# hpcaitech/Open-Sora

Hardware: NVIDIA H100
Metric: denoise-steps/sec STDiT3-XL/2 64x32x32 bf16 (higher is better)
Workload: dtype bf16

## Files before the change

open-sora_b200/csrc/attn_sm90.cu:

```cuda
#include <stdlib.h>

#include "common.cuh"
#include "stage.cuh"
#include "tiles.cuh"
#include "wgmma.cuh"

namespace osb {

constexpr int kAttnThreads = 256;
constexpr int kKeyBlock = 64;

template <int D>
struct FlashState {
  static constexpr int DP = HeadTileCfg<D>::DP;
  uint32_t q[DP / 16][4];
  float o[DP / 8][4];
  float m[2], l[2];
};

template <int D>
__device__ __forceinline__ void flash_load_q(FlashState<D>& f, uint32_t sq, uint32_t chunk_bytes) {
  using Cfg = HeadTileCfg<D>;
  const int lane = threadIdx.x & 31, warp = threadIdx.x >> 5;
  const int row = warp * 16 + (lane & 15);
#pragma unroll
  for (int kk = 0; kk < Cfg::DP / 16; ++kk)
    ldsm_x4(sq + tile_unit_off<Cfg::MAIN>(row, 2 * kk + (lane >> 4), chunk_bytes), f.q[kk][0], f.q[kk][1], f.q[kk][2], f.q[kk][3]);
#pragma unroll
  for (int j = 0; j < Cfg::DP / 8; ++j) f.o[j][0] = f.o[j][1] = f.o[j][2] = f.o[j][3] = 0.f;
  f.m[0] = f.m[1] = -INFINITY;
  f.l[0] = f.l[1] = 0.f;
}

template <int D, bool kBias = false>
__device__ __forceinline__ void flash_block(FlashState<D>& f, uint32_t sk, uint32_t sv, uint32_t chunk_bytes, int krow0,
                                            int n16, int key0, const int (&lo)[2], const int (&hi)[2], float sc,
                                            const float* bias = nullptr, int boff0 = 0, int boff1 = 0, float bscale = 0.f) {
  using Cfg = HeadTileCfg<D>;
  constexpr int NB = kKeyBlock / 8;
  const int lane = threadIdx.x & 31;
  float s[NB][4];
#pragma unroll
  for (int g = 0; g < kKeyBlock / 16; ++g) {
    s[2 * g][0] = s[2 * g][1] = s[2 * g][2] = s[2 * g][3] = 0.f;
    s[2 * g + 1][0] = s[2 * g + 1][1] = s[2 * g + 1][2] = s[2 * g + 1][3] = 0.f;
    if (g >= n16) continue;
    const int krow = krow0 + g * 16 + (lane & 7) + ((lane >> 4) << 3);
#pragma unroll
    for (int kk = 0; kk < Cfg::DP / 16; ++kk) {
      uint32_t b0, b1, b2, b3;
      ldsm_x4(sk + tile_unit_off<Cfg::MAIN>(krow, 2 * kk + ((lane >> 3) & 1), chunk_bytes), b0, b1, b2, b3);
      mma_bf16_16816(s[2 * g], f.q[kk], b0, b1);
      mma_bf16_16816(s[2 * g + 1], f.q[kk], b2, b3);
    }
  }
  float mx[2] = {-INFINITY, -INFINITY};
#pragma unroll
  for (int j = 0; j < NB; ++j) {
#pragma unroll
    for (int e = 0; e < 4; ++e) {
      const int i = e >> 1;
      const int key = key0 + 8 * j + 2 * (lane & 3) + (e & 1);
      if (j >= 2 * n16 || key < lo[i] || key >= hi[i]) s[j][e] = -INFINITY;
      else if constexpr (kBias) s[j][e] = fmaf(s[j][e], bscale, __ldg(bias + key + (i ? boff1 : boff0)));
      mx[i] = fmaxf(mx[i], s[j][e]);
    }
  }
  float alpha[2], ms[2];
#pragma unroll
  for (int i = 0; i < 2; ++i) {
    mx[i] = fmaxf(mx[i], __shfl_xor_sync(0xffffffffu, mx[i], 1));
    mx[i] = fmaxf(mx[i], __shfl_xor_sync(0xffffffffu, mx[i], 2));
    const float mn = fmaxf(f.m[i], mx[i]);
    alpha[i] = (mn == -INFINITY) ? 1.f : fast_exp2((f.m[i] - mn) * sc);
    ms[i] = (mn == -INFINITY) ? 0.f : mn * sc;
    f.m[i] = mn;
    f.l[i] *= alpha[i];
  }
#pragma unroll
  for (int j = 0; j < Cfg::DP / 8; ++j) {
    f.o[j][0] *= alpha[0]; f.o[j][1] *= alpha[0];
    f.o[j][2] *= alpha[1]; f.o[j][3] *= alpha[1];
  }
#pragma unroll
  for (int j = 0; j < NB; ++j) {
#pragma unroll
    for (int e = 0; e < 4; ++e) {
      s[j][e] = fast_exp2(fmaf(s[j][e], sc, -ms[e >> 1]));
      f.l[e >> 1] += s[j][e];
    }
  }
#pragma unroll
  for (int g = 0; g < kKeyBlock / 16; ++g) {
    if (g >= n16) continue;
    const uint32_t a[4] = {pack_bf16x2(s[2 * g][0], s[2 * g][1]), pack_bf16x2(s[2 * g][2], s[2 * g][3]),
                           pack_bf16x2(s[2 * g + 1][0], s[2 * g + 1][1]), pack_bf16x2(s[2 * g + 1][2], s[2 * g + 1][3])};
    const int vrow = krow0 + g * 16 + (lane & 7) + (((lane >> 3) & 1) << 3);
#pragma unroll
    for (int dg = 0; dg < Cfg::DP / 16; ++dg) {
      uint32_t b0, b1, b2, b3;
      ldsm_x4_t(sv + tile_unit_off<Cfg::MAIN>(vrow, 2 * dg + (lane >> 4), chunk_bytes), b0, b1, b2, b3);
      mma_bf16_16816(f.o[2 * dg], a, b0, b1);
      mma_bf16_16816(f.o[2 * dg + 1], a, b2, b3);
    }
  }
}

template <int D>
__device__ __forceinline__ void flash_store(FlashState<D>& f, __nv_bfloat16* dst0, __nv_bfloat16* dst1) {
  const int lane = threadIdx.x & 31;
  float inv[2];
#pragma unroll
  for (int i = 0; i < 2; ++i) {
    float l = f.l[i];
    l += __shfl_xor_sync(0xffffffffu, l, 1);
    l += __shfl_xor_sync(0xffffffffu, l, 2);
    inv[i] = l > 0.f ? 1.0f / l : 0.f;
  }
#pragma unroll
  for (int j = 0; j < D / 8; ++j) {
    const int c = 8 * j + 2 * (lane & 3);
    if (dst0) *reinterpret_cast<uint32_t*>(dst0 + c) = pack_bf16x2(f.o[j][0] * inv[0], f.o[j][1] * inv[0]);
    if (dst1) *reinterpret_cast<uint32_t*>(dst1 + c) = pack_bf16x2(f.o[j][2] * inv[1], f.o[j][3] * inv[1]);
  }
}

struct TileAttnParams {
  const uint8_t* q; const uint8_t* k; const uint8_t* v;
  int64_t q_head_stride, kv_head_stride;
  int32_t q_tile_bytes, kv_tile_bytes;
  int64_t items;
  float scale_log2;
  TileSets ts;
};

template <int D>
struct TileAttnSmem {
  static constexpr int kSlot = 128 * HeadTileCfg<D>::ROW_BYTES;
  static constexpr int kStages = D == 128 ? 2 : (D == 72 ? 4 : 5);
  static constexpr int kData = 2 * kSlot + kStages * 2 * kSlot;
  static constexpr int kBytes = 1024 + kData + 8 * (4 + 2 * kStages);
  static_assert(kBytes <= 227 * 1024 && 2 * kBytes > 228 * 1024, "one resident CTA per SM");
};

constexpr int kTileAttnThreads = 384;

template <int D>
__global__ void __launch_bounds__(kTileAttnThreads, 1) attn_tiles_kernel(const TileAttnParams p) {
  using Cfg = HeadTileCfg<D>;
  using Sm = TileAttnSmem<D>;
  constexpr int MAIN = Cfg::MAIN, TAIL = Cfg::TAIL, STAGES = Sm::kStages;
  extern __shared__ uint8_t smem_raw[];
  const uint32_t base = (smem_u32(smem_raw) + 1023u) & ~1023u;
  auto sQ = [&](int b) { return base + (uint32_t)(b * Sm::kSlot); };
  auto sK = [&](int s) { return base + (uint32_t)((2 + 2 * s) * Sm::kSlot); };
  auto sV = [&](int s) { return sK(s) + (uint32_t)Sm::kSlot; };
  const uint32_t bar = base + (uint32_t)Sm::kData;
  auto q_full = [&](int b) { return bar + 8u * b; };
  auto q_empty = [&](int b) { return bar + 16u + 8u * b; };
  auto full_bar = [&](int s) { return bar + 32u + 8u * s; };
  auto empty_bar = [&](int s) { return bar + 32u + 8u * (STAGES + s); };

  const int wg = threadIdx.x >> 7, tid_wg = threadIdx.x & 127;
  const int64_t begin = (int64_t)blockIdx.x * p.items / gridDim.x, end = (int64_t)(blockIdx.x + 1) * p.items / gridDim.x;
  const TileSets& ts = p.ts;
  const int tps = ts.qmap.tps;

  {
    uint4* z = reinterpret_cast<uint4*>(smem_raw + (base - smem_u32(smem_raw)));
    for (int i = threadIdx.x; i < Sm::kData / 16; i += kTileAttnThreads) z[i] = make_uint4(0, 0, 0, 0);
  }
  fence_proxy_async_smem();
  if (threadIdx.x == 0) {
    for (int b = 0; b < 2; ++b) { mbar_init(q_full(b), 1); mbar_init(q_empty(b), 2); }
    for (int s = 0; s < STAGES; ++s) { mbar_init(full_bar(s), 1); mbar_init(empty_bar(s), 2); }
    fence_barrier_init();
  }
  __syncthreads();
  pdl_wait();

  if (wg == 0) {
    asm volatile("setmaxnreg.dec.sync.aligned.u32 40;\n" ::: "memory");
    if (tid_wg == 0) {
      uint32_t kv_it = 0;
      for (int64_t it = begin; it < end; ++it) {
        const uint32_t n = (uint32_t)(it - begin);
        const int64_t hs = it / tps, head = hs / ts.num_sets, set = hs - head * ts.num_sets;
        const int qs = n & 1;
        mbar_wait_notrace(q_empty(qs), ((n >> 1) & 1u) ^ 1u);
        mbar_expect_tx(q_full(qs), (uint32_t)p.q_tile_bytes);
        bulk_load_1d(sQ(qs), p.q + head * p.q_head_stride + (it - head * ts.num_sets * tps) * p.q_tile_bytes,
                     (uint32_t)p.q_tile_bytes, q_full(qs));
        const int nkt = (tile_set_keys(ts, set) + ts.BK - 1) / ts.BK;
        if (it > begin && (it - 1) / tps == hs && nkt <= STAGES) continue;
        const int64_t off = head * p.kv_head_stride + set * ts.nkb * (int64_t)p.kv_tile_bytes;
        for (int t = 0; t < nkt; ++t, ++kv_it) {
          const int s = (int)(kv_it % STAGES);
          mbar_wait_notrace(empty_bar(s), ((kv_it / STAGES) & 1u) ^ 1u);
          mbar_expect_tx(full_bar(s), 2u * (uint32_t)p.kv_tile_bytes);
          bulk_load_1d(sK(s), p.k + off + (int64_t)t * p.kv_tile_bytes, (uint32_t)p.kv_tile_bytes, full_bar(s));
          bulk_load_1d(sV(s), p.v + off + (int64_t)t * p.kv_tile_bytes, (uint32_t)p.kv_tile_bytes, full_bar(s));
        }
      }
      pdl_launch_dependents();
    }
    return;
  }

  asm volatile("setmaxnreg.inc.sync.aligned.u32 232;\n" ::: "memory");
  const int cw = wg - 1;
  const int lane = tid_wg & 31, quad = lane & 3;
  const int r_loc = cw * 64 + (tid_wg >> 5) * 16 + (lane >> 2);
  const float sc = p.scale_log2;
  float s[64], o[MAIN][32], ot[TAIL ? 8 : 1];
#pragma unroll
  for (int i = 0; i < 64; ++i) s[i] = 0.f;
  uint32_t kv_it = 0, kv0 = 0;
  for (int64_t it = begin; it < end; ++it) {
    const uint32_t n = (uint32_t)(it - begin);
    const int64_t hs = it / tps, head = hs / ts.num_sets, set = hs - head * ts.num_sets;
    const int qt = (int)(it - hs * tps), qs = n & 1;
    const int keys = tile_set_keys(ts, set);
    const int nkt = (keys + ts.BK - 1) / ts.BK;
    if (!(it > begin && (it - 1) / tps == hs && nkt <= STAGES)) { kv0 = kv_it; kv_it += nkt; }
    const bool keep = it + 1 < end && (it + 1) / tps == hs && nkt <= STAGES;

    int64_t seq[2];
    int pos[2], lo[2], hi[2];
    bool valid[2];
#pragma unroll
    for (int hh = 0; hh < 2; ++hh) tile_query_row(ts, set, qt, keys, r_loc + 8 * hh, seq[hh], pos[hh], valid[hh], lo[hh], hi[hh]);
#pragma unroll
    for (int c = 0; c < MAIN; ++c)
#pragma unroll
      for (int i = 0; i < 32; ++i) o[c][i] = 0.f;
#pragma unroll
    for (int i = 0; i < (TAIL ? 8 : 1); ++i) ot[i] = 0.f;
    float m[2] = {-INFINITY, -INFINITY}, l[2] = {0.f, 0.f};

    const uint32_t q_chunk = (uint32_t)ts.qmap.TR * 128u, kv_chunk = (uint32_t)ts.BK * 128u;
    const uint32_t qa = sQ(qs) + (uint32_t)(cw * 64 * 128), qa_tail = sQ(qs) + MAIN * q_chunk + (uint32_t)(cw * 8 * 256);
    mbar_wait_notrace(q_full(qs), (n >> 1) & 1u);
    for (int t = 0; t < nkt; ++t) {
      const uint32_t u = kv0 + (uint32_t)t;
      const int st = (int)(u % STAGES);
      mbar_wait_notrace(full_bar(st), (u / STAGES) & 1u);
      const uint32_t ka = sK(st), va = sV(st);
      wgmma_fence_regs(s);
      wgmma_fence();
#pragma unroll
      for (int c = 0; c < MAIN; ++c)
#pragma unroll
        for (int k = 0; k < 4; ++k)
          Wgmma<128>::mma(s, make_sw128_kmajor_desc(qa + c * q_chunk + 32u * k),
                          make_sw128_kmajor_desc(ka + c * kv_chunk + 32u * k), (c | k) ? 1u : 0u);
      if constexpr (TAIL != 0)
        Wgmma<128>::mma(s, make_noswizzle_desc(qa_tail, 128u, 256u), make_noswizzle_desc(ka + MAIN * kv_chunk, 128u, 256u), 1u);
      wgmma_commit();
      wgmma_wait<0>();
      wgmma_fence_regs(s);
      if (t == nkt - 1 && tid_wg == 0) mbar_arrive(q_empty(qs));
      const int slot0 = t * ts.BK;
      const int n16 = ((keys - slot0 < ts.BK ? keys - slot0 : ts.BK) + 15) >> 4;
      float mx[2] = {-INFINITY, -INFINITY};
#pragma unroll
      for (int i = 0; i < 64; ++i) {
        const int hh = (i >> 1) & 1;
        const int col = 8 * (i >> 2) + 2 * quad + (i & 1), key = slot0 + col;
        if (col >= ts.BK || key < lo[hh] || key >= hi[hh]) s[i] = -INFINITY;
        mx[hh] = fmaxf(mx[hh], s[i]);
      }
      float alpha[2], ms[2];
#pragma unroll
      for (int hh = 0; hh < 2; ++hh) {
        mx[hh] = fmaxf(mx[hh], __shfl_xor_sync(0xffffffffu, mx[hh], 1));
        mx[hh] = fmaxf(mx[hh], __shfl_xor_sync(0xffffffffu, mx[hh], 2));
        const float mn = fmaxf(m[hh], mx[hh]);
        alpha[hh] = (mn == -INFINITY) ? 1.f : fast_exp2((m[hh] - mn) * sc);
        ms[hh] = (mn == -INFINITY) ? 0.f : mn * sc;
        m[hh] = mn;
        l[hh] *= alpha[hh];
      }
#pragma unroll
      for (int c = 0; c < MAIN; ++c)
#pragma unroll
        for (int i = 0; i < 32; ++i) o[c][i] *= alpha[(i >> 1) & 1];
      if constexpr (TAIL != 0) {
#pragma unroll
        for (int i = 0; i < 8; ++i) ot[i] *= alpha[(i >> 1) & 1];
      }
      uint32_t pa[8][4];
#pragma unroll
      for (int i = 0; i < 64; ++i) {
        s[i] = (i >> 3) < n16 ? fast_exp2(fmaf(s[i], sc, -ms[(i >> 1) & 1])) : 0.f;
        l[(i >> 1) & 1] += s[i];
      }
#pragma unroll
      for (int g = 0; g < 8; ++g) {
        pa[g][0] = pack_bf16x2(s[8 * g + 0], s[8 * g + 1]);
        pa[g][1] = pack_bf16x2(s[8 * g + 2], s[8 * g + 3]);
        pa[g][2] = pack_bf16x2(s[8 * g + 4], s[8 * g + 5]);
        pa[g][3] = pack_bf16x2(s[8 * g + 6], s[8 * g + 7]);
      }
#pragma unroll
      for (int c = 0; c < MAIN; ++c) wgmma_fence_regs(o[c]);
      if constexpr (TAIL != 0) wgmma_fence_regs(ot);
      wgmma_fence();
#pragma unroll
      for (int g = 0; g < 8; ++g) {
#pragma unroll
        for (int c = 0; c < MAIN; ++c)
          WgmmaRegAT<64>::mma(o[c], pa[g], make_sw128_kmajor_desc(va + c * kv_chunk + 2048u * g), 1u);
        if constexpr (TAIL != 0)
          WgmmaRegAT<16>::mma(ot, pa[g], make_noswizzle_desc(va + MAIN * kv_chunk + 512u * g, 256u, 128u), 1u);
      }
      wgmma_commit();
      wgmma_wait<0>();
#pragma unroll
      for (int c = 0; c < MAIN; ++c) wgmma_fence_regs(o[c]);
      if constexpr (TAIL != 0) wgmma_fence_regs(ot);
#pragma unroll
      for (int g = 0; g < 8; ++g) fence_regs_u32(pa[g]);
      if (!keep && tid_wg == 0) mbar_arrive(empty_bar(st));
    }
    if (nkt == 0 && tid_wg == 0) mbar_arrive(q_empty(qs));

#pragma unroll
    for (int hh = 0; hh < 2; ++hh) {
      float lt = l[hh];
      lt += __shfl_xor_sync(0xffffffffu, lt, 1);
      lt += __shfl_xor_sync(0xffffffffu, lt, 2);
      const float inv = lt > 0.f ? 1.0f / lt : 0.f;
      if (!valid[hh]) continue;
      __nv_bfloat16* dst = tile_out_row(ts, seq[hh], pos[hh]) + head * D + 2 * quad;
#pragma unroll
      for (int c = 0; c < MAIN; ++c)
#pragma unroll
        for (int j = 0; j < 8; ++j)
          *reinterpret_cast<uint32_t*>(dst + 64 * c + 8 * j) = pack_bf16x2(o[c][4 * j + 2 * hh] * inv, o[c][4 * j + 2 * hh + 1] * inv);
      if constexpr (TAIL != 0)
        *reinterpret_cast<uint32_t*>(dst + 64 * MAIN) = pack_bf16x2(ot[2 * hh] * inv, ot[2 * hh + 1] * inv);
    }
  }
}

template <int D>
static int attn_tiles_launch(TileAttnParams& p, int H, cudaStream_t stream) {
  using Cfg = HeadTileCfg<D>;
  p.q_tile_bytes = p.ts.qmap.TR * Cfg::ROW_BYTES;
  p.kv_tile_bytes = p.ts.BK * Cfg::ROW_BYTES;
  p.items = (int64_t)H * p.ts.num_sets * p.ts.qmap.tps;
  if (p.items >= (1ll << 31)) { set_error("osb_attn_tiles: problem too large (%lld work items)", (long long)p.items); return OSB_ERR_UNSUPPORTED; }
  const int64_t grid = p.items < sm_count() ? p.items : sm_count();
  cudaLaunchAttribute attr[2];
  cudaLaunchConfig_t cfg = launch_config(dim3((unsigned)grid), dim3(kTileAttnThreads), TileAttnSmem<D>::kBytes, stream, attr);
  OSB_CHECK_CUDA(cudaLaunchKernelEx(&cfg, attn_tiles_kernel<D>, p));
  count_launch();
  return OSB_OK;
}

struct AttnParams {
  const __nv_bfloat16* q; const __nv_bfloat16* k; const __nv_bfloat16* v; __nv_bfloat16* out;
  int64_t q_ld, k_ld, v_ld, out_ld;
  int64_t num_seqs, seqs_per_batch;
  int64_t q_bs, q_ss, q_ts, k_bs, k_ss, k_ts;
  int32_t Lq, Lk;
  const int32_t* kv_lens;
  const __nv_bfloat16* qw; const __nv_bfloat16* kw;
  const __nv_bfloat16* qw2; const __nv_bfloat16* kw2;
  int32_t norm_split;
  float eps;
  const float* cos; const float* sin;
  int32_t rope_half;
  float scale_log2;
  int32_t G;
  int32_t tiles_per_seq;
  const float* bias;
  int64_t bias_hs;
  float scale;
};

template <int D>
__device__ __forceinline__ void stage_row(uint4 (&raw)[HeadTileCfg<D>::U], bool norm, float eps, const __nv_bfloat16* w,
                                          const float* cosr, const float* sinr, bool rope_half, uint8_t* tile,
                                          uint32_t chunk_bytes, int row) {
  using Cfg = HeadTileCfg<D>;
  constexpr int U = Cfg::U;
  norm_rope_row<D, U>(raw, norm, eps, w, cosr, sinr, rope_half);
#pragma unroll
  for (int u = 0; u < Cfg::UP; ++u)
    *reinterpret_cast<uint4*>(tile + tile_unit_off<Cfg::MAIN>(row, u, chunk_bytes)) = u < U ? raw[u] : make_uint4(0, 0, 0, 0);
}

template <int D, bool kBias>
__global__ void __launch_bounds__(kAttnThreads, 1) attn_short_kernel(const AttnParams p) {
  using Cfg = HeadTileCfg<D>;
  constexpr int U = Cfg::U;
  extern __shared__ __align__(1024) uint8_t smem[];
  uint8_t* sQ = smem;
  uint8_t* sK = smem + 128 * Cfg::ROW_BYTES;
  uint8_t* sV = sK + kKeyBlock * Cfg::ROW_BYTES;
  const int tid = threadIdx.x, lane = tid & 31, warp = tid >> 5;
  const int64_t unit = blockIdx.x;
  const int h = blockIdx.y;

  int64_t seq0;
  int qt = 0;
  if (p.G > 1) seq0 = unit * p.G;
  else { seq0 = unit / p.tiles_per_seq; qt = (int)(unit - seq0 * p.tiles_per_seq); }
  auto row_of = [&](int64_t seq, int tok, int64_t bs, int64_t ss, int64_t ts) {
    const int64_t b = seq / p.seqs_per_batch, j = seq - b * p.seqs_per_batch;
    return b * bs + j * ss + (int64_t)tok * ts;
  };

  __shared__ int s_nkeys;
  if (tid == 0) s_nkeys = 0;
  __syncthreads();
  pdl_wait();
  for (int r = tid; r < 128; r += kAttnThreads) {
    const int g = p.G > 1 ? r / p.Lq : 0;
    const int tok = p.G > 1 ? r - g * p.Lq : qt * 128 + r;
    const int64_t seq = seq0 + g;
    uint4 raw[U];
    const bool ok = g < p.G && seq < p.num_seqs && tok < p.Lq;
    if (ok) {
      const uint4* src = reinterpret_cast<const uint4*>(p.q + row_of(seq, tok, p.q_bs, p.q_ss, p.q_ts) * p.q_ld + (int64_t)h * D);
#pragma unroll
      for (int u = 0; u < U; ++u) raw[u] = __ldg(src + u);
    } else {
#pragma unroll
      for (int u = 0; u < U; ++u) raw[u] = make_uint4(0, 0, 0, 0);
    }
    const __nv_bfloat16* w = (p.qw2 != nullptr && tok >= p.norm_split) ? p.qw2 : p.qw;
    const bool rope = ok && p.cos != nullptr;
    stage_row<D>(raw, ok && p.qw != nullptr, p.eps, w, rope ? p.cos + (int64_t)tok * (D / 2) : nullptr,
                 rope ? p.sin + (int64_t)tok * (D / 2) : nullptr, p.rope_half, sQ, 128u * 128u, r);
  }

  int lo[2], hi[2];
  int boff[2] = {0, 0};
  __nv_bfloat16* dst[2] = {nullptr, nullptr};
  int nkeys = 0;
#pragma unroll
  for (int i = 0; i < 2; ++i) {
    const int r = warp * 16 + (lane >> 2) + 8 * i;
    const int g = p.G > 1 ? r / p.Lq : 0;
    const int tok = p.G > 1 ? r - g * p.Lq : qt * 128 + r;
    const int64_t seq = seq0 + g;
    lo[i] = hi[i] = 0;
    if (g < p.G && seq < p.num_seqs && tok < p.Lq) {
      int len = p.kv_lens ? p.kv_lens[seq] : p.Lk;
      len = len < p.Lk ? (len < 0 ? 0 : len) : p.Lk;
      lo[i] = g * p.Lk;
      hi[i] = lo[i] + len;
      if constexpr (kBias) boff[i] = p.Lq - 1 - tok - lo[i];
      dst[i] = p.out + row_of(seq, tok, p.q_bs, p.q_ss, p.q_ts) * p.out_ld + (int64_t)h * D;
    }
    nkeys = hi[i] > nkeys ? hi[i] : nkeys;
  }
  atomicMax(&s_nkeys, nkeys);
  __syncthreads();
  nkeys = s_nkeys;

  FlashState<D> f;
  flash_load_q<D>(f, smem_u32(sQ), 128u * 128u);
  const float sc = p.scale_log2;
  const float* bh = nullptr;
  if constexpr (kBias) bh = p.bias + (int64_t)h * p.bias_hs;
  for (int k0 = 0; k0 < nkeys; k0 += kKeyBlock) {
    if constexpr (kBias) {
      if (p.G == 1) {
        const int iq0 = qt * 128, iq1 = (iq0 + 128 < p.Lq ? iq0 + 128 : p.Lq) - 1;
        const int kend = k0 + kKeyBlock < nkeys ? k0 + kKeyBlock : nkeys;
        const int d0 = k0 - iq1 + p.Lq - 1, d1 = kend - 1 - iq0 + p.Lq - 1;
        const bool live = d0 + tid <= d1 && __ldg(bh + d0 + tid) != -INFINITY;
// ... 209 lines not shown
```

open-sora_b200/csrc/wgmma.cuh:

```cuda
#pragma once

#include <stdint.h>

namespace osb {

template <int N>
struct Wgmma;

template <>
struct Wgmma<64> {
  static constexpr int kRegs = 32;
  __device__ __forceinline__ static void mma(float (&d)[32], uint64_t da, uint64_t db, uint32_t accumulate) {
    asm volatile(
        "{\n\t.reg .pred p;\n\tsetp.ne.b32 p, %34, 0;\n\t"
        "wgmma.mma_async.sync.aligned.m64n64k16.f32.bf16.bf16 "
        "{%0, %1, %2, %3, %4, %5, %6, %7, %8, %9, %10, %11, %12, %13, %14, %15, %16, %17, %18, %19, %20, %21, %22, %23, %24, %25, %26, %27, %28, %29, %30, %31}, "
        "%32, %33, p, 1, 1, 0, 0;\n\t}\n"
        : "+f"(d[0]), "+f"(d[1]), "+f"(d[2]), "+f"(d[3]), "+f"(d[4]), "+f"(d[5]), "+f"(d[6]), "+f"(d[7]),
        "+f"(d[8]), "+f"(d[9]), "+f"(d[10]), "+f"(d[11]), "+f"(d[12]), "+f"(d[13]), "+f"(d[14]), "+f"(d[15]),
        "+f"(d[16]), "+f"(d[17]), "+f"(d[18]), "+f"(d[19]), "+f"(d[20]), "+f"(d[21]), "+f"(d[22]), "+f"(d[23]),
        "+f"(d[24]), "+f"(d[25]), "+f"(d[26]), "+f"(d[27]), "+f"(d[28]), "+f"(d[29]), "+f"(d[30]), "+f"(d[31])
        : "l"(da), "l"(db), "r"(accumulate));
  }
};

template <>
struct Wgmma<128> {
  static constexpr int kRegs = 64;
  __device__ __forceinline__ static void mma(float (&d)[64], uint64_t da, uint64_t db, uint32_t accumulate) {
    asm volatile(
        "{\n\t.reg .pred p;\n\tsetp.ne.b32 p, %66, 0;\n\t"
        "wgmma.mma_async.sync.aligned.m64n128k16.f32.bf16.bf16 "
        "{%0, %1, %2, %3, %4, %5, %6, %7, %8, %9, %10, %11, %12, %13, %14, %15, %16, %17, %18, %19, %20, %21, %22, %23, %24, %25, %26, %27, %28, %29, %30, %31, %32, %33, %34, %35, %36, %37, %38, %39, %40, %41, %42, %43, %44, %45, %46, %47, %48, %49, %50, %51, %52, %53, %54, %55, %56, %57, %58, %59, %60, %61, %62, %63}, "
        "%64, %65, p, 1, 1, 0, 0;\n\t}\n"
        : "+f"(d[0]), "+f"(d[1]), "+f"(d[2]), "+f"(d[3]), "+f"(d[4]), "+f"(d[5]), "+f"(d[6]), "+f"(d[7]),
        "+f"(d[8]), "+f"(d[9]), "+f"(d[10]), "+f"(d[11]), "+f"(d[12]), "+f"(d[13]), "+f"(d[14]), "+f"(d[15]),
        "+f"(d[16]), "+f"(d[17]), "+f"(d[18]), "+f"(d[19]), "+f"(d[20]), "+f"(d[21]), "+f"(d[22]), "+f"(d[23]),
        "+f"(d[24]), "+f"(d[25]), "+f"(d[26]), "+f"(d[27]), "+f"(d[28]), "+f"(d[29]), "+f"(d[30]), "+f"(d[31]),
        "+f"(d[32]), "+f"(d[33]), "+f"(d[34]), "+f"(d[35]), "+f"(d[36]), "+f"(d[37]), "+f"(d[38]), "+f"(d[39]),
        "+f"(d[40]), "+f"(d[41]), "+f"(d[42]), "+f"(d[43]), "+f"(d[44]), "+f"(d[45]), "+f"(d[46]), "+f"(d[47]),
        "+f"(d[48]), "+f"(d[49]), "+f"(d[50]), "+f"(d[51]), "+f"(d[52]), "+f"(d[53]), "+f"(d[54]), "+f"(d[55]),
        "+f"(d[56]), "+f"(d[57]), "+f"(d[58]), "+f"(d[59]), "+f"(d[60]), "+f"(d[61]), "+f"(d[62]), "+f"(d[63])
        : "l"(da), "l"(db), "r"(accumulate));
  }
};

template <>
struct Wgmma<144> {
  static constexpr int kRegs = 72;
  __device__ __forceinline__ static void mma(float (&d)[72], uint64_t da, uint64_t db, uint32_t accumulate) {
    asm volatile(
        "{\n\t.reg .pred p;\n\tsetp.ne.b32 p, %74, 0;\n\t"
        "wgmma.mma_async.sync.aligned.m64n144k16.f32.bf16.bf16 "
        "{%0, %1, %2, %3, %4, %5, %6, %7, %8, %9, %10, %11, %12, %13, %14, %15, %16, %17, %18, %19, %20, %21, %22, %23, %24, %25, %26, %27, %28, %29, %30, %31, %32, %33, %34, %35, %36, %37, %38, %39, %40, %41, %42, %43, %44, %45, %46, %47, %48, %49, %50, %51, %52, %53, %54, %55, %56, %57, %58, %59, %60, %61, %62, %63, %64, %65, %66, %67, %68, %69, %70, %71}, "
        "%72, %73, p, 1, 1, 0, 0;\n\t}\n"
        : "+f"(d[0]), "+f"(d[1]), "+f"(d[2]), "+f"(d[3]), "+f"(d[4]), "+f"(d[5]), "+f"(d[6]), "+f"(d[7]),
        "+f"(d[8]), "+f"(d[9]), "+f"(d[10]), "+f"(d[11]), "+f"(d[12]), "+f"(d[13]), "+f"(d[14]), "+f"(d[15]),
        "+f"(d[16]), "+f"(d[17]), "+f"(d[18]), "+f"(d[19]), "+f"(d[20]), "+f"(d[21]), "+f"(d[22]), "+f"(d[23]),
        "+f"(d[24]), "+f"(d[25]), "+f"(d[26]), "+f"(d[27]), "+f"(d[28]), "+f"(d[29]), "+f"(d[30]), "+f"(d[31]),
        "+f"(d[32]), "+f"(d[33]), "+f"(d[34]), "+f"(d[35]), "+f"(d[36]), "+f"(d[37]), "+f"(d[38]), "+f"(d[39]),
        "+f"(d[40]), "+f"(d[41]), "+f"(d[42]), "+f"(d[43]), "+f"(d[44]), "+f"(d[45]), "+f"(d[46]), "+f"(d[47]),
        "+f"(d[48]), "+f"(d[49]), "+f"(d[50]), "+f"(d[51]), "+f"(d[52]), "+f"(d[53]), "+f"(d[54]), "+f"(d[55]),
        "+f"(d[56]), "+f"(d[57]), "+f"(d[58]), "+f"(d[59]), "+f"(d[60]), "+f"(d[61]), "+f"(d[62]), "+f"(d[63]),
        "+f"(d[64]), "+f"(d[65]), "+f"(d[66]), "+f"(d[67]), "+f"(d[68]), "+f"(d[69]), "+f"(d[70]), "+f"(d[71])
        : "l"(da), "l"(db), "r"(accumulate));
  }
};

template <>
struct Wgmma<192> {
  static constexpr int kRegs = 96;
  __device__ __forceinline__ static void mma(float (&d)[96], uint64_t da, uint64_t db, uint32_t accumulate) {
    asm volatile(
        "{\n\t.reg .pred p;\n\tsetp.ne.b32 p, %98, 0;\n\t"
        "wgmma.mma_async.sync.aligned.m64n192k16.f32.bf16.bf16 "
        "{%0, %1, %2, %3, %4, %5, %6, %7, %8, %9, %10, %11, %12, %13, %14, %15, %16, %17, %18, %19, %20, %21, %22, %23, %24, %25, %26, %27, %28, %29, %30, %31, %32, %33, %34, %35, %36, %37, %38, %39, %40, %41, %42, %43, %44, %45, %46, %47, %48, %49, %50, %51, %52, %53, %54, %55, %56, %57, %58, %59, %60, %61, %62, %63, %64, %65, %66, %67, %68, %69, %70, %71, %72, %73, %74, %75, %76, %77, %78, %79, %80, %81, %82, %83, %84, %85, %86, %87, %88, %89, %90, %91, %92, %93, %94, %95}, "
        "%96, %97, p, 1, 1, 0, 0;\n\t}\n"
        : "+f"(d[0]), "+f"(d[1]), "+f"(d[2]), "+f"(d[3]), "+f"(d[4]), "+f"(d[5]), "+f"(d[6]), "+f"(d[7]),
        "+f"(d[8]), "+f"(d[9]), "+f"(d[10]), "+f"(d[11]), "+f"(d[12]), "+f"(d[13]), "+f"(d[14]), "+f"(d[15]),
        "+f"(d[16]), "+f"(d[17]), "+f"(d[18]), "+f"(d[19]), "+f"(d[20]), "+f"(d[21]), "+f"(d[22]), "+f"(d[23]),
        "+f"(d[24]), "+f"(d[25]), "+f"(d[26]), "+f"(d[27]), "+f"(d[28]), "+f"(d[29]), "+f"(d[30]), "+f"(d[31]),
        "+f"(d[32]), "+f"(d[33]), "+f"(d[34]), "+f"(d[35]), "+f"(d[36]), "+f"(d[37]), "+f"(d[38]), "+f"(d[39]),
        "+f"(d[40]), "+f"(d[41]), "+f"(d[42]), "+f"(d[43]), "+f"(d[44]), "+f"(d[45]), "+f"(d[46]), "+f"(d[47]),
        "+f"(d[48]), "+f"(d[49]), "+f"(d[50]), "+f"(d[51]), "+f"(d[52]), "+f"(d[53]), "+f"(d[54]), "+f"(d[55]),
        "+f"(d[56]), "+f"(d[57]), "+f"(d[58]), "+f"(d[59]), "+f"(d[60]), "+f"(d[61]), "+f"(d[62]), "+f"(d[63]),
        "+f"(d[64]), "+f"(d[65]), "+f"(d[66]), "+f"(d[67]), "+f"(d[68]), "+f"(d[69]), "+f"(d[70]), "+f"(d[71]),
        "+f"(d[72]), "+f"(d[73]), "+f"(d[74]), "+f"(d[75]), "+f"(d[76]), "+f"(d[77]), "+f"(d[78]), "+f"(d[79]),
        "+f"(d[80]), "+f"(d[81]), "+f"(d[82]), "+f"(d[83]), "+f"(d[84]), "+f"(d[85]), "+f"(d[86]), "+f"(d[87]),
        "+f"(d[88]), "+f"(d[89]), "+f"(d[90]), "+f"(d[91]), "+f"(d[92]), "+f"(d[93]), "+f"(d[94]), "+f"(d[95])
        : "l"(da), "l"(db), "r"(accumulate));
  }
};

template <>
struct Wgmma<256> {
  static constexpr int kRegs = 128;
  __device__ __forceinline__ static void mma(float (&d)[128], uint64_t da, uint64_t db, uint32_t accumulate) {
    asm volatile(
        "{\n\t.reg .pred p;\n\tsetp.ne.b32 p, %130, 0;\n\t"
        "wgmma.mma_async.sync.aligned.m64n256k16.f32.bf16.bf16 "
        "{%0, %1, %2, %3, %4, %5, %6, %7, %8, %9, %10, %11, %12, %13, %14, %15, %16, %17, %18, %19, %20, %21, %22, %23, %24, %25, %26, %27, %28, %29, %30, %31, %32, %33, %34, %35, %36, %37, %38, %39, %40, %41, %42, %43, %44, %45, %46, %47, %48, %49, %50, %51, %52, %53, %54, %55, %56, %57, %58, %59, %60, %61, %62, %63, %64, %65, %66, %67, %68, %69, %70, %71, %72, %73, %74, %75, %76, %77, %78, %79, %80, %81, %82, %83, %84, %85, %86, %87, %88, %89, %90, %91, %92, %93, %94, %95, %96, %97, %98, %99, %100, %101, %102, %103, %104, %105, %106, %107, %108, %109, %110, %111, %112, %113, %114, %115, %116, %117, %118, %119, %120, %121, %122, %123, %124, %125, %126, %127}, "
        "%128, %129, p, 1, 1, 0, 0;\n\t}\n"
        : "+f"(d[0]), "+f"(d[1]), "+f"(d[2]), "+f"(d[3]), "+f"(d[4]), "+f"(d[5]), "+f"(d[6]), "+f"(d[7]),
        "+f"(d[8]), "+f"(d[9]), "+f"(d[10]), "+f"(d[11]), "+f"(d[12]), "+f"(d[13]), "+f"(d[14]), "+f"(d[15]),
        "+f"(d[16]), "+f"(d[17]), "+f"(d[18]), "+f"(d[19]), "+f"(d[20]), "+f"(d[21]), "+f"(d[22]), "+f"(d[23]),
        "+f"(d[24]), "+f"(d[25]), "+f"(d[26]), "+f"(d[27]), "+f"(d[28]), "+f"(d[29]), "+f"(d[30]), "+f"(d[31]),
        "+f"(d[32]), "+f"(d[33]), "+f"(d[34]), "+f"(d[35]), "+f"(d[36]), "+f"(d[37]), "+f"(d[38]), "+f"(d[39]),
        "+f"(d[40]), "+f"(d[41]), "+f"(d[42]), "+f"(d[43]), "+f"(d[44]), "+f"(d[45]), "+f"(d[46]), "+f"(d[47]),
        "+f"(d[48]), "+f"(d[49]), "+f"(d[50]), "+f"(d[51]), "+f"(d[52]), "+f"(d[53]), "+f"(d[54]), "+f"(d[55]),
        "+f"(d[56]), "+f"(d[57]), "+f"(d[58]), "+f"(d[59]), "+f"(d[60]), "+f"(d[61]), "+f"(d[62]), "+f"(d[63]),
        "+f"(d[64]), "+f"(d[65]), "+f"(d[66]), "+f"(d[67]), "+f"(d[68]), "+f"(d[69]), "+f"(d[70]), "+f"(d[71]),
        "+f"(d[72]), "+f"(d[73]), "+f"(d[74]), "+f"(d[75]), "+f"(d[76]), "+f"(d[77]), "+f"(d[78]), "+f"(d[79]),
        "+f"(d[80]), "+f"(d[81]), "+f"(d[82]), "+f"(d[83]), "+f"(d[84]), "+f"(d[85]), "+f"(d[86]), "+f"(d[87]),
        "+f"(d[88]), "+f"(d[89]), "+f"(d[90]), "+f"(d[91]), "+f"(d[92]), "+f"(d[93]), "+f"(d[94]), "+f"(d[95]),
        "+f"(d[96]), "+f"(d[97]), "+f"(d[98]), "+f"(d[99]), "+f"(d[100]), "+f"(d[101]), "+f"(d[102]), "+f"(d[103]),
        "+f"(d[104]), "+f"(d[105]), "+f"(d[106]), "+f"(d[107]), "+f"(d[108]), "+f"(d[109]), "+f"(d[110]), "+f"(d[111]),
        "+f"(d[112]), "+f"(d[113]), "+f"(d[114]), "+f"(d[115]), "+f"(d[116]), "+f"(d[117]), "+f"(d[118]), "+f"(d[119]),
        "+f"(d[120]), "+f"(d[121]), "+f"(d[122]), "+f"(d[123]), "+f"(d[124]), "+f"(d[125]), "+f"(d[126]), "+f"(d[127])
        : "l"(da), "l"(db), "r"(accumulate));
  }
};

template <int N>
struct WgmmaBT;
template <>
struct WgmmaBT<64> {
  __device__ __forceinline__ static void mma(float (&d)[32], uint64_t da, uint64_t db, uint32_t accumulate) {
    asm volatile(
        "{\n\t.reg .pred p;\n\tsetp.ne.b32 p, %34, 0;\n\t"
        "wgmma.mma_async.sync.aligned.m64n64k16.f32.bf16.bf16 "
        "{%0, %1, %2, %3, %4, %5, %6, %7, %8, %9, %10, %11, %12, %13, %14, %15, %16, %17, %18, %19, %20, %21, %22, %23, %24, %25, %26, %27, %28, %29, %30, %31}, "
        "%32, %33, p, 1, 1, 0, 1;\n\t}\n"
        : "+f"(d[0]), "+f"(d[1]), "+f"(d[2]), "+f"(d[3]), "+f"(d[4]), "+f"(d[5]), "+f"(d[6]), "+f"(d[7]),
        "+f"(d[8]), "+f"(d[9]), "+f"(d[10]), "+f"(d[11]), "+f"(d[12]), "+f"(d[13]), "+f"(d[14]), "+f"(d[15]),
        "+f"(d[16]), "+f"(d[17]), "+f"(d[18]), "+f"(d[19]), "+f"(d[20]), "+f"(d[21]), "+f"(d[22]), "+f"(d[23]),
        "+f"(d[24]), "+f"(d[25]), "+f"(d[26]), "+f"(d[27]), "+f"(d[28]), "+f"(d[29]), "+f"(d[30]), "+f"(d[31])
        : "l"(da), "l"(db), "r"(accumulate));
  }
};

__device__ __forceinline__ uint64_t make_noswizzle_desc(uint32_t smem_addr, uint32_t lbo, uint32_t sbo) {
  uint64_t d = 0;
  d |= static_cast<uint64_t>((smem_addr & 0x3FFFF) >> 4);
  d |= static_cast<uint64_t>(lbo >> 4) << 16;
  d |= static_cast<uint64_t>(sbo >> 4) << 32;
  return d;
}

template <int N>
struct WgmmaRegAT;
template <>
struct WgmmaRegAT<64> {
  __device__ __forceinline__ static void mma(float (&d)[32], const uint32_t (&a)[4], uint64_t db, uint32_t accumulate) {
    asm volatile(
        "{\n\t.reg .pred p;\n\tsetp.ne.b32 p, %37, 0;\n\t"
        "wgmma.mma_async.sync.aligned.m64n64k16.f32.bf16.bf16 "
        "{%0, %1, %2, %3, %4, %5, %6, %7, %8, %9, %10, %11, %12, %13, %14, %15, %16, %17, %18, %19, %20, %21, %22, %23, %24, %25, %26, %27, %28, %29, %30, %31}, "
        "{%32, %33, %34, %35}, %36, p, 1, 1, 1;\n\t}\n"
        : "+f"(d[0]), "+f"(d[1]), "+f"(d[2]), "+f"(d[3]), "+f"(d[4]), "+f"(d[5]), "+f"(d[6]), "+f"(d[7]),
        "+f"(d[8]), "+f"(d[9]), "+f"(d[10]), "+f"(d[11]), "+f"(d[12]), "+f"(d[13]), "+f"(d[14]), "+f"(d[15]),
// ... 164 lines not shown
```

Baseline: 12.02.

## Size attention wgmma N to valid keys and skip masking for full blocks

The SM90 tile attention consumer now picks the wgmma N width (16/32/64/128) from the number of valid keys in each key block. For windowed layouts, each consumer warpgroup computes only its own 64-key half. This avoids QK^T and PV tensor-core work and exp work on padded or out-of-window keys. A fast path also skips per-element mask checks when a whole block is in range, and 32-bit index math replaces 64-bit divisions. The cost is more template instantiations and code size, and the window path assumes each warpgroup's queries only attend to its matching 64 keys.

```diff
diff --git a/open-sora_b200/csrc/attn_sm90.cu b/open-sora_b200/csrc/attn_sm90.cu
--- a/open-sora_b200/csrc/attn_sm90.cu
+++ b/open-sora_b200/csrc/attn_sm90.cu
@@ -1,4 +1,6 @@
 #include <stdlib.h>
+
+#include <type_traits>
 
 #include "common.cuh"
 #include "stage.cuh"
@@ -185,14 +187,15 @@
       uint32_t kv_it = 0;
       for (int64_t it = begin; it < end; ++it) {
         const uint32_t n = (uint32_t)(it - begin);
-        const int64_t hs = it / tps, head = hs / ts.num_sets, set = hs - head * ts.num_sets;
-        const int qs = n & 1;
+        const uint32_t hs = (uint32_t)it / (uint32_t)tps, head32 = hs / (uint32_t)ts.num_sets;
+        const int64_t head = head32, set = hs - head32 * (uint32_t)ts.num_sets;
+        const int qt = (int)((uint32_t)it - hs * (uint32_t)tps), qs = n & 1;
         mbar_wait_notrace(q_empty(qs), ((n >> 1) & 1u) ^ 1u);
         mbar_expect_tx(q_full(qs), (uint32_t)p.q_tile_bytes);
         bulk_load_1d(sQ(qs), p.q + head * p.q_head_stride + (it - head * ts.num_sets * tps) * p.q_tile_bytes,
                      (uint32_t)p.q_tile_bytes, q_full(qs));
         const int nkt = (tile_set_keys(ts, set) + ts.BK - 1) / ts.BK;
-        if (it > begin && (it - 1) / tps == hs && nkt <= STAGES) continue;
+        if (it > begin && qt > 0 && nkt <= STAGES) continue;
         const int64_t off = head * p.kv_head_stride + set * ts.nkb * (int64_t)p.kv_tile_bytes;
         for (int t = 0; t < nkt; ++t, ++kv_it) {
           const int s = (int)(kv_it % STAGES);
@@ -212,18 +215,18 @@
   const int lane = tid_wg & 31, quad = lane & 3;
   const int r_loc = cw * 64 + (tid_wg >> 5) * 16 + (lane >> 2);
   const float sc = p.scale_log2;
-  float s[64], o[MAIN][32], ot[TAIL ? 8 : 1];
-#pragma unroll
-  for (int i = 0; i < 64; ++i) s[i] = 0.f;
+  const bool window = ts.qmap.G > 1 && 64 % ts.qmap.L == 0 && ts.Lk == ts.qmap.L;
+  float o[MAIN][32], ot[TAIL ? 8 : 1];
   uint32_t kv_it = 0, kv0 = 0;
   for (int64_t it = begin; it < end; ++it) {
     const uint32_t n = (uint32_t)(it - begin);
-    const int64_t hs = it / tps, head = hs / ts.num_sets, set = hs - head * ts.num_sets;
-    const int qt = (int)(it - hs * tps), qs = n & 1;
+    const uint32_t hs = (uint32_t)it / (uint32_t)tps, head32 = hs / (uint32_t)ts.num_sets;
+    const int64_t head = head32, set = hs - head32 * (uint32_t)ts.num_sets;
+    const int qt = (int)((uint32_t)it - hs * (uint32_t)tps), qs = n & 1;
     const int keys = tile_set_keys(ts, set);
     const int nkt = (keys + ts.BK - 1) / ts.BK;
-    if (!(it > begin && (it - 1) / tps == hs && nkt <= STAGES)) { kv0 = kv_it; kv_it += nkt; }
-    const bool keep = it + 1 < end && (it + 1) / tps == hs && nkt <= STAGES;
+    if (!(it > begin && qt > 0 && nkt <= STAGES)) { kv0 = kv_it; kv_it += nkt; }
+    const bool keep = it + 1 < end && qt + 1 < tps && nkt <= STAGES;
 
     int64_t seq[2];
     int pos[2], lo[2], hi[2];
@@ -245,82 +248,110 @@
       const uint32_t u = kv0 + (uint32_t)t;
       const int st = (int)(u % STAGES);
       mbar_wait_notrace(full_bar(st), (u / STAGES) & 1u);
-      const uint32_t ka = sK(st), va = sV(st);
-      wgmma_fence_regs(s);
-      wgmma_fence();
-#pragma unroll
-      for (int c = 0; c < MAIN; ++c)
-#pragma unroll
-        for (int k = 0; k < 4; ++k)
-          Wgmma<128>::mma(s, make_sw128_kmajor_desc(qa + c * q_chunk + 32u * k),
+      const int slot0 = t * ts.BK;
+      const int nvalid = keys - slot0 < ts.BK ? keys - slot0 : ts.BK;
+      const int n16 = (nvalid + 15) >> 4;
+      auto step = [&](auto width, const int koff) {
+        constexpr int N = decltype(width)::value, NR = N / 2, KS = N / 16;
+        const uint32_t ka = sK(st) + (uint32_t)koff * 128u, va = sV(st) + (uint32_t)koff * 128u;
+        const uint32_t ka_tail = sK(st) + MAIN * kv_chunk + (uint32_t)koff * 32u, va_tail = sV(st) + MAIN * kv_chunk + (uint32_t)koff * 32u;
+        float s[NR];
+#pragma unroll
+        for (int i = 0; i < NR; ++i) s[i] = 0.f;
+        wgmma_fence_regs(s);
+        wgmma_fence();
+#pragma unroll
+        for (int c = 0; c < MAIN; ++c)
+#pragma unroll
+          for (int k = 0; k < 4; ++k)
+            Wgmma<N>::mma(s, make_sw128_kmajor_desc(qa + c * q_chunk + 32u * k),
                           make_sw128_kmajor_desc(ka + c * kv_chunk + 32u * k), (c | k) ? 1u : 0u);
-      if constexpr (TAIL != 0)
-        Wgmma<128>::mma(s, make_noswizzle_desc(qa_tail, 128u, 256u), make_noswizzle_desc(ka + MAIN * kv_chunk, 128u, 256u), 1u);
-      wgmma_commit();
-      wgmma_wait<0>();
-      wgmma_fence_regs(s);
-      if (t == nkt - 1 && tid_wg == 0) mbar_arrive(q_empty(qs));
-      const int slot0 = t * ts.BK;
-      const int n16 = ((keys - slot0 < ts.BK ? keys - slot0 : ts.BK) + 15) >> 4;
-      float mx[2] = {-INFINITY, -INFINITY};
-#pragma unroll
-      for (int i = 0; i < 64; ++i) {
-        const int hh = (i >> 1) & 1;
-        const int col = 8 * (i >> 2) + 2 * quad + (i & 1), key = slot0 + col;
-        if (col >= ts.BK || key < lo[hh] || key >= hi[hh]) s[i] = -INFINITY;
-        mx[hh] = fmaxf(mx[hh], s[i]);
-      }
-      float alpha[2], ms[2];
-#pragma unroll
-      for (int hh = 0; hh < 2; ++hh) {
-        mx[hh] = fmaxf(mx[hh], __shfl_xor_sync(0xffffffffu, mx[hh], 1));
-        mx[hh] = fmaxf(mx[hh], __shfl_xor_sync(0xffffffffu, mx[hh], 2));
-        const float mn = fmaxf(m[hh], mx[hh]);
-        alpha[hh] = (mn == -INFINITY) ? 1.f : fast_exp2((m[hh] - mn) * sc);
-        ms[hh] = (mn == -INFINITY) ? 0.f : mn * sc;
-        m[hh] = mn;
-        l[hh] *= alpha[hh];
-      }
-#pragma unroll
-      for (int c = 0; c < MAIN; ++c)
-#pragma unroll
-        for (int i = 0; i < 32; ++i) o[c][i] *= alpha[(i >> 1) & 1];
-      if constexpr (TAIL != 0) {
-#pragma unroll
-        for (int i = 0; i < 8; ++i) ot[i] *= alpha[(i >> 1) & 1];
-      }
-      uint32_t pa[8][4];
-#pragma unroll
-      for (int i = 0; i < 64; ++i) {
-        s[i] = (i >> 3) < n16 ? fast_exp2(fmaf(s[i], sc, -ms[(i >> 1) & 1])) : 0.f;
-        l[(i >> 1) & 1] += s[i];
-      }
-#pragma unroll
-      for (int g = 0; g < 8; ++g) {
-        pa[g][0] = pack_bf16x2(s[8 * g + 0], s[8 * g + 1]);
-        pa[g][1] = pack_bf16x2(s[8 * g + 2], s[8 * g + 3]);
-        pa[g][2] = pack_bf16x2(s[8 * g + 4], s[8 * g + 5]);
-        pa[g][3] = pack_bf16x2(s[8 * g + 6], s[8 * g + 7]);
-      }
-#pragma unroll
-      for (int c = 0; c < MAIN; ++c) wgmma_fence_regs(o[c]);
-      if constexpr (TAIL != 0) wgmma_fence_regs(ot);
-      wgmma_fence();
-#pragma unroll
-      for (int g = 0; g < 8; ++g) {
+        if constexpr (TAIL != 0)
+          Wgmma<N>::mma(s, make_noswizzle_desc(qa_tail, 128u, 256u), make_noswizzle_desc(ka_tail, 128u, 256u), 1u);
+        wgmma_commit();
+        wgmma_wait<0>();
+        wgmma_fence_regs(s);
+        if (t == nkt - 1 && tid_wg == 0) mbar_arrive(q_empty(qs));
+        const int k0 = slot0 + koff;
+        const bool all_in = koff + N <= nvalid && k0 >= lo[0] && k0 + N <= hi[0] && k0 >= lo[1] && k0 + N <= hi[1];
+        float mx[2] = {-INFINITY, -INFINITY};
+        if (all_in) {
+#pragma unroll
+          for (int i = 0; i < NR; ++i) mx[(i >> 1) & 1] = fmaxf(mx[(i >> 1) & 1], s[i]);
+        } else {
+#pragma unroll
+          for (int i = 0; i < NR; ++i) {
+            const int hh = (i >> 1) & 1;
+            const int col = koff + 8 * (i >> 2) + 2 * quad + (i & 1), key = slot0 + col;
+            if (col >= ts.BK || key < lo[hh] || key >= hi[hh]) s[i] = -INFINITY;
+            mx[hh] = fmaxf(mx[hh], s[i]);
+          }
+        }
+        float alpha[2], ms[2];
+#pragma unroll
+        for (int hh = 0; hh < 2; ++hh) {
+          mx[hh] = fmaxf(mx[hh], __shfl_xor_sync(0xffffffffu, mx[hh], 1));
+          mx[hh] = fmaxf(mx[hh], __shfl_xor_sync(0xffffffffu, mx[hh], 2));
+          const float mn = fmaxf(m[hh], mx[hh]);
+          alpha[hh] = (mn == -INFINITY) ? 1.f : fast_exp2((m[hh] - mn) * sc);
+          ms[hh] = (mn == -INFINITY) ? 0.f : mn * sc;
+          m[hh] = mn;
+          l[hh] = __fmul_rn(l[hh], alpha[hh]);
+        }
 #pragma unroll
         for (int c = 0; c < MAIN; ++c)
-          WgmmaRegAT<64>::mma(o[c], pa[g], make_sw128_kmajor_desc(va + c * kv_chunk + 2048u * g), 1u);
-        if constexpr (TAIL != 0)
-          WgmmaRegAT<16>::mma(ot, pa[g], make_noswizzle_desc(va + MAIN * kv_chunk + 512u * g, 256u, 128u), 1u);
-      }
-      wgmma_commit();
-      wgmma_wait<0>();
-#pragma unroll
-      for (int c = 0; c < MAIN; ++c) wgmma_fence_regs(o[c]);
-      if constexpr (TAIL != 0) wgmma_fence_regs(ot);
-#pragma unroll
-      for (int g = 0; g < 8; ++g) fence_regs_u32(pa[g]);
+#pragma unroll
+          for (int i = 0; i < 32; ++i) o[c][i] *= alpha[(i >> 1) & 1];
+        if constexpr (TAIL != 0) {
+#pragma unroll
+          for (int i = 0; i < 8; ++i) ot[i] *= alpha[(i >> 1) & 1];
+        }
+        uint32_t pa[KS][4];
+        if (all_in) {
+#pragma unroll
+          for (int i = 0; i < NR; ++i) {
+            s[i] = fast_exp2(fmaf(s[i], sc, -ms[(i >> 1) & 1]));
+            l[(i >> 1) & 1] += s[i];
+          }
+        } else {
+#pragma unroll
+          for (int i = 0; i < NR; ++i) {
+            s[i] = (koff >> 4) + (i >> 3) < n16 ? fast_exp2(fmaf(s[i], sc, -ms[(i >> 1) & 1])) : 0.f;
+            l[(i >> 1) & 1] += s[i];
+          }
+        }
+#pragma unroll
+        for (int g = 0; g < KS; ++g) {
+          pa[g][0] = pack_bf16x2(s[8 * g + 0], s[8 * g + 1]);
+          pa[g][1] = pack_bf16x2(s[8 * g + 2], s[8 * g + 3]);
+          pa[g][2] = pack_bf16x2(s[8 * g + 4], s[8 * g + 5]);
+          pa[g][3] = pack_bf16x2(s[8 * g + 6], s[8 * g + 7]);
+        }
+#pragma unroll
+        for (int c = 0; c < MAIN; ++c) wgmma_fence_regs(o[c]);
+        if constexpr (TAIL != 0) wgmma_fence_regs(ot);
+        wgmma_fence();
+#pragma unroll
+        for (int g = 0; g < KS; ++g) {
+#pragma unroll
+          for (int c = 0; c < MAIN; ++c)
+            WgmmaRegAT<64>::mma(o[c], pa[g], make_sw128_kmajor_desc(va + c * kv_chunk + 2048u * g), 1u);
+          if constexpr (TAIL != 0)
+            WgmmaRegAT<16>::mma(ot, pa[g], make_noswizzle_desc(va_tail + 512u * g, 256u, 128u), 1u);
+        }
+        wgmma_commit();
+        wgmma_wait<0>();
+#pragma unroll
+        for (int c = 0; c < MAIN; ++c) wgmma_fence_regs(o[c]);
+        if constexpr (TAIL != 0) wgmma_fence_regs(ot);
+#pragma unroll
+        for (int g = 0; g < KS; ++g) fence_regs_u32(pa[g]);
+      };
+      if (window) step(std::integral_constant<int, 64>{}, 64 * cw);
+      else if (nvalid <= 16) step(std::integral_constant<int, 16>{}, 0);
+      else if (nvalid <= 32) step(std::integral_constant<int, 32>{}, 0);
+      else if (nvalid <= 64) step(std::integral_constant<int, 64>{}, 0);
+      else step(std::integral_constant<int, 128>{}, 0);
       if (!keep && tid_wg == 0) mbar_arrive(empty_bar(st));
     }
     if (nkt == 0 && tid_wg == 0) mbar_arrive(q_empty(qs));
diff --git a/open-sora_b200/csrc/wgmma.cuh b/open-sora_b200/csrc/wgmma.cuh
--- a/open-sora_b200/csrc/wgmma.cuh
+++ b/open-sora_b200/csrc/wgmma.cuh
@@ -6,6 +6,35 @@
 
 template <int N>
 struct Wgmma;
+
+template <>
+struct Wgmma<16> {
+  static constexpr int kRegs = 8;
+  __device__ __forceinline__ static void mma(float (&d)[8], uint64_t da, uint64_t db, uint32_t accumulate) {
+    asm volatile(
+        "{\n\t.reg .pred p;\n\tsetp.ne.b32 p, %10, 0;\n\t"
+        "wgmma.mma_async.sync.aligned.m64n16k16.f32.bf16.bf16 "
+        "{%0, %1, %2, %3, %4, %5, %6, %7}, "
+        "%8, %9, p, 1, 1, 0, 0;\n\t}\n"
+        : "+f"(d[0]), "+f"(d[1]), "+f"(d[2]), "+f"(d[3]), "+f"(d[4]), "+f"(d[5]), "+f"(d[6]), "+f"(d[7])
+        : "l"(da), "l"(db), "r"(accumulate));
+  }
+};
+
+template <>
+struct Wgmma<32> {
+  static constexpr int kRegs = 16;
+  __device__ __forceinline__ static void mma(float (&d)[16], uint64_t da, uint64_t db, uint32_t accumulate) {
+    asm volatile(
+        "{\n\t.reg .pred p;\n\tsetp.ne.b32 p, %18, 0;\n\t"
+        "wgmma.mma_async.sync.aligned.m64n32k16.f32.bf16.bf16 "
+        "{%0, %1, %2, %3, %4, %5, %6, %7, %8, %9, %10, %11, %12, %13, %14, %15}, "
+        "%16, %17, p, 1, 1, 0, 0;\n\t}\n"
+        : "+f"(d[0]), "+f"(d[1]), "+f"(d[2]), "+f"(d[3]), "+f"(d[4]), "+f"(d[5]), "+f"(d[6]), "+f"(d[7]),
+        "+f"(d[8]), "+f"(d[9]), "+f"(d[10]), "+f"(d[11]), "+f"(d[12]), "+f"(d[13]), "+f"(d[14]), "+f"(d[15])
+        : "l"(da), "l"(db), "r"(accumulate));
+  }
+};
 
 template <>
 struct Wgmma<64> {
```

Measured after the change: 12.35 (median of 6 runs). +2.7%, better.
